# youmi-zym/GO-SLAM

Measured on NVIDIA H100. Metric: keyframe-BA-updates/s, higher is better.
Workload: dtype f16 corr (f32 accumulate) / f32 BA (f64 solve)

## Files before the change

### go-slam_b200/csrc/ba.cu

```cuda
#include "common.cuh"
#include <cstring>
#include "se3.cuh"
#include <algorithm>
#include <cstdio>
#include <mutex>
#include <cooperative_groups.h>

namespace {

constexpr int kTP = 128;
constexpr int kNRed = 27;
constexpr float kAlpha = 0.05f;

struct BaWs {
  int* slot_of_frame;
  int* kx;
  int* counts;
  int* row_ptr;
  int* edge_idx;
  int* entry_ptr;
  int* entry_code;
  int* pair_ptr;
  int* edge_j;
  float* Eij;
// ... 178 lines not shown

__device__ __forceinline__ float warp_transpose_reduce32(float (&v)[32], int lane) {
  transpose_reduce_step<16>(v, lane);
  return v[0];
}

struct BaIn {
  const float* poses; const float* disps; const float* intr; const float* disps_sens;
  const float* targets; const float* weights; const float* eta; int eta_rows;
  const int64_t* ii; const int64_t* jj;
};

__device__ __forceinline__ void linearize_tile(const BaIn& in, const BaDims& d, const BaWs& ws,
                                               int motion_only, int k, int wt) {
  const float* poses = in.poses; const float* disps = in.disps;
  const float* __restrict__ intr = in.intr; const float* __restrict__ disps_sens = in.disps_sens;
  const float* __restrict__ targets = in.targets; const float* __restrict__ weights = in.weights;
  const float* __restrict__ eta = in.eta; const int eta_rows = in.eta_rows;
  const int f = ws.kx[k];
  const int lane = threadIdx.x & 31;
  const int px = wt * 32 + lane;
  const bool act = px < d.hw;

  const float fx = intr[0], fy = intr[1], cx = intr[2], cy = intr[3];
  const float u = (float)(px % d.wd), v = (float)(px / d.wd);
  const float di = act ? disps[(size_t)f * d.hw + px] : 1.0f;
  float Xi[4] = {(u - cx) / fx, (v - cy) / fy, 1.0f, di};

  float C = 0.f, wz = 0.f;
  float Ei[6] = {0.f, 0.f, 0.f, 0.f, 0.f, 0.f};

  const int r0 = ws.row_ptr[f], r1 = ws.row_ptr[f + 1];
  float pi[7];
#pragma unroll
  for (int c = 0; c < 7; ++c) pi[c] = poses[7 * (size_t)f + c];
  int e1 = 0, j1 = f, e2 = 0, j2 = f;
  if (r0 < r1) { e1 = ws.edge_idx[r0]; j1 = ws.edge_j[e1]; }
  if (r0 + 1 < r1) { e2 = ws.edge_idx[r0 + 1]; j2 = ws.edge_j[e2]; }
  float nx[4] = {0.f, 0.f, 0.f, 0.f}, pn[7] = {0.f, 0.f, 0.f, 0.f, 0.f, 0.f, 1.f};
  if (r0 < r1) {
    if (act) {
      const size_t o = ((size_t)e1 * 2) * d.hw + px;
      nx[0] = targets[o]; nx[1] = targets[o + d.hw]; nx[2] = weights[o]; nx[3] = weights[o + d.hw];
    }
#pragma unroll
    for (int c = 0; c < 7; ++c) pn[c] = poses[7 * (size_t)j1 + c];
  }
  for (int r = r0; r < r1; ++r) {
    const int e = e1, jx = j1;
    const float tu = nx[0], tv = nx[1], qu = nx[2], qv = nx[3];
    float pj[7];
#pragma unroll
    for (int c = 0; c < 7; ++c) pj[c] = pn[c];
    e1 = e2; j1 = j2;
    if (r + 1 < r1) {
      if (act) {
        const size_t o = ((size_t)e1 * 2) * d.hw + px;
        nx[0] = targets[o]; nx[1] = targets[o + d.hw]; nx[2] = weights[o]; nx[3] = weights[o + d.hw];
      }
#pragma unroll
      for (int c = 0; c < 7; ++c) pn[c] = poses[7 * (size_t)j1 + c];
    }
    if (r + 2 < r1) { e2 = ws.edge_idx[r + 2]; j2 = ws.edge_j[e2]; }
    const bool stereo = (jx == f);
    GsSE3 G;
    if (stereo) {
      G.t[0] = -0.1f; G.t[1] = 0.f; G.t[2] = 0.f;
      G.q[0] = 0.f; G.q[1] = 0.f; G.q[2] = 0.f; G.q[3] = 1.f;
    } else {
      gs_rel(pi, pi + 3, pj, pj + 3, G);
    }

    float Xj[4];
    gs_act4(G, Xi, Xj);
    const float x = Xj[0], y = Xj[1], h = Xj[3];
    const bool behind = Xj[2] < GS_MIN_DEPTH;
    const float dd = behind ? 0.0f : __frcp_rn(Xj[2]);
    const float d2 = dd * dd;
    float wu = (behind || !act) ? 0.0f : (float)(.001 * (double)qu);
    float wv = (behind || !act) ? 0.0f : (float)(.001 * (double)qv);
    const float ru = tu - (fx * dd * x + cx);
    const float rv = tv - (fy * dd * y + cy);

    float Ju[6], Jv[6];
    Ju[0] = fx * (h * dd);       Ju[1] = fx * 0.f;
    Ju[2] = fx * (-x * h * d2);  Ju[3] = fx * (-x * y * d2);
    Ju[4] = fx * (1 + x * x * d2);  Ju[5] = fx * (-y * dd);
    Jv[0] = fy * 0.f;            Jv[1] = fy * (h * dd);
    Jv[2] = fy * (-y * h * d2);  Jv[3] = fy * (-1 - y * y * d2);
    Jv[4] = fy * (x * y * d2);   Jv[5] = fy * (x * dd);
    const float Jzu = fx * (G.t[0] * dd - G.t[2] * (x * d2));
    const float Jzv = fy * (G.t[1] * dd - G.t[2] * (y * d2));

    C += wu * Jzu * Jzu;  C += wv * Jzv * Jzv;
    wz += wu * ru * Jzu;  wz += wv * rv * Jzv;
    if (stereo) { wu = 0.f; wv = 0.f; }

    float val[32];
    {
      int l = 0;
#pragma unroll
      for (int a = 0; a < 6; ++a)
#pragma unroll
        for (int b = a; b < 6; ++b) val[l++] = wu * Ju[a] * Ju[b] + wv * Jv[a] * Jv[b];
#pragma unroll
      for (int a = 0; a < 6; ++a) val[21 + a] = wu * ru * Ju[a] + wv * rv * Jv[a];
#pragma unroll
      for (int a = kNRed; a < 32; ++a) val[a] = 0.f;
    }
    const float tot = warp_transpose_reduce32(val, lane);
    if (lane < kNRed)
      ws.part[((size_t)e * ws.ntiles * (kTP / 32) + wt) * kNRed + lane] = tot;

    if (!motion_only) {
      float Ee[6], Eii[6];
#pragma unroll
      for (int a = 0; a < 6; ++a) Ee[a] = wu * Jzu * Ju[a] + wv * Jzv * Jv[a];
      gs_adjT(G, Ee, Eii);
      if (act) {
#pragma unroll
        for (int a = 0; a < 6; ++a) {
          ws.Eij[((size_t)e * 6 + a) * d.hw + px] = Ee[a];
          Ei[a] -= Eii[a];
        }
      }
    }
  }

  if (!motion_only && act) {
    const float ds = disps_sens[(size_t)f * d.hw + px];
    const float m = (ds > 0.f) ? 1.0f : 0.0f;
    const int er = (eta_rows == 1) ? 0 : (eta_rows < 0 ? f : k);
    const float et = eta[(size_t)er * d.hw + px];
    C = C + m * kAlpha + (1.0f - m) * et;
    wz = wz - m * kAlpha * (di - ds);
    const size_t o = (size_t)k * d.hw + px;
    ws.Q[o] = 1.0f / C;
    ws.w[o] = wz;
#pragma unroll
    for (int a = 0; a < 6; ++a) ws.Ei[((size_t)k * 6 + a) * d.hw + px] = Ei[a];
  }
}

__global__ void __launch_bounds__(kTP)
ba_linearize_kernel(BaIn in, BaDims d, BaWs ws, int motion_only) {
  if ((int)blockIdx.y >= ws.counts[0] || ws.counts[4]) return;
  linearize_tile(in, d, ws, motion_only, blockIdx.y, blockIdx.x * (kTP / 32) + (threadIdx.x >> 5));
}

struct SysSmem {
  float red[8][64];
  double redd[8][32];
  double Hs[36], Ms[36], Ts[36], vs[6];
};

template <int NT>
__device__ __forceinline__ void system_items(const float* poses, const int64_t* __restrict__ ii,
                                             const int64_t* __restrict__ jj, const BaDims& d,
                                             const BaWs& ws, double* sys, int motion_only, int bid,
                                             int nb, SysSmem& sm) {
  float (*red)[64] = sm.red;
  double* Hs = sm.Hs; double* Ms = sm.Ms; double* Ts = sm.Ts; double* vs = sm.vs;
  const int tid = threadIdx.x, lane = tid & 31, warp = tid >> 5;
  const int M = ws.counts[0];
  const int npairs = motion_only ? 0 : ws.counts[2];
  constexpr int kChunk = 4 * NT;
  const int nchunk = (d.hw + kChunk - 1) / kChunk;
  double* H = sys;
  double* bvec = sys + (size_t)d.n * d.n;

  for (int e = nb - 1 - bid; e < d.N; e += nb) {
    const int ix = (int)ii[e], jx = (int)jj[e];
    const int pi = ix - d.t0, pj = jx - d.t0;
    const bool vi_ok = pi >= 0 && pi < d.P, vj_ok = pj >= 0 && pj < d.P;
    if ((!vi_ok && !vj_ok) || ix < 0 || ix >= d.num) continue;
    {
      double ps = 0.0;
      if (lane < kNRed) {
        const int nparts = ws.ntiles * (kTP / 32);
        const float* pp = ws.part + (size_t)e * nparts * kNRed + lane;
#pragma unroll 8
        for (int t = warp; t < nparts; t += NT / 32) ps += (double)pp[(size_t)t * kNRed];
      }
      sm.redd[warp][lane] = ps;
    }
    __syncthreads();
    if (tid < kNRed) {
      double s = 0.0;
#pragma unroll
      for (int wq = 0; wq < NT / 32; ++wq) s += sm.redd[wq][tid];
      if (tid < 21) {
        int a = 0, l = tid;
        while (l >= 6 - a) { l -= 6 - a; ++a; }
        const int b = a + l;
        Hs[a * 6 + b] = s; Hs[b * 6 + a] = s;
      } else {
        vs[tid - 21] = s;
      }
    }
    if (tid >= 32 && tid < 38) {
      const int c = tid - 32;
      GsSE3 G;
      gs_edge_pose(poses, ix, jx, G);
      float X[6], Y[6];
#pragma unroll
      for (int r = 0; r < 6; ++r) X[r] = (r == c) ? 1.0f : 0.0f;
      gs_adjT(G, X, Y);
#pragma unroll
      for (int r = 0; r < 6; ++r) Ms[r * 6 + c] = (double)Y[r];
    }
    __syncthreads();
    if (tid < 36) {
      const int r = tid / 6, c = tid % 6;
      double s = 0.0;
      for (int q = 0; q < 6; ++q) s += Ms[r * 6 + q] * Hs[q * 6 + c];
      Ts[tid] = s;
    }
    __syncthreads();
    if (tid < 36) {
      const int r = tid / 6, c = tid % 6;
      if (vi_ok) {
        double s = 0.0;
        for (int q = 0; q < 6; ++q) s += Ts[r * 6 + q] * Ms[c * 6 + q];
        atomicAdd(&H[(size_t)(6 * pi + r) * d.n + 6 * pi + c], s);
      }
      if (vi_ok && vj_ok) {
        atomicAdd(&H[(size_t)(6 * pi + r) * d.n + 6 * pj + c], -Ts[r * 6 + c]);
        atomicAdd(&H[(size_t)(6 * pj + r) * d.n + 6 * pi + c], -Ts[c * 6 + r]);
      }
      if (vj_ok) atomicAdd(&H[(size_t)(6 * pj + r) * d.n + 6 * pj + c], Hs[r * 6 + c]);
    } else if (tid >= 64 && tid < 70) {
      const int r = tid - 64;
      if (vj_ok) atomicAdd(&bvec[6 * pj + r], vs[r]);
      if (vi_ok) {
        double s = 0.0;
        for (int q = 0; q < 6; ++q) s += Ms[r * 6 + q] * vs[q];
        atomicAdd(&bvec[6 * pi + r], -s);
      }
    }
    __syncthreads();
  }

  const int total = npairs * nchunk;
  const int per = (total + nb - 1) / nb;
  const int u0 = bid * per;
  const int u1 = min(total, u0 + per);
  int cur = -1, pa = 0, pb = 0;
  bool diag = false;
  const float* Ea = nullptr; const float* Eb = nullptr; const float* Qk = nullptr; const float* wk = nullptr;
  float acc[64];
  auto flush = [&]() {
    float lo32[32], hi32[32];
#pragma unroll
    for (int i = 0; i < 32; ++i) { lo32[i] = acc[i]; hi32[i] = acc[32 + i]; }
    const float s0 = warp_transpose_reduce32(lo32, lane);
    const float s1 = warp_transpose_reduce32(hi32, lane);
    red[warp][lane] = s0;
    red[warp][32 + lane] = s1;
    __syncthreads();
    if (tid < 42) {
      double s = 0.0;
#pragma unroll
      for (int wq = 0; wq < NT / 32; ++wq) s += (double)red[wq][tid];
      if (tid < 36) {
        const int r = tid / 6, c = tid % 6;
        atomicAdd(&H[(size_t)(6 * pa + r) * d.n + 6 * pb + c], -s);
        if (!diag) atomicAdd(&H[(size_t)(6 * pb + c) * d.n + 6 * pa + r], -s);
      } else {
        atomicAdd(&bvec[6 * pa + (tid - 36)], -s);
      }
    }
    __syncthreads();
  };
  for (int u = u0; u < u1; ++u) {
    const int p = u / nchunk;
    const int px0 = (u - p * nchunk) * kChunk;
    const int px1 = min(d.hw, px0 + kChunk);
    if (p != cur) {
      if (cur >= 0) flush();
      cur = p;
      int k;
      if (M <= 32) {
        const int v = lane < M ? ws.pair_ptr[lane] : 0x7fffffff;
        k = __popc(__ballot_sync(0xffffffffu, v <= p)) - 1;
      } else {
        int lo = 0, hi = M;
        while (hi - lo > 1) {
          const int mid = (lo + hi) >> 1;
          if (ws.pair_ptr[mid] <= p) lo = mid; else hi = mid;
        }
        k = lo;
      }
      const int e0 = ws.entry_ptr[k];
      const int ne = ws.entry_ptr[k + 1] - e0;
      int q = p - ws.pair_ptr[k];
      int a = 0;
      while (q >= ne - a) { q -= ne - a; ++a; }
      const int b = a + q;
      const int ca = ws.entry_code[e0 + a];
      const int cb = ws.entry_code[e0 + b];
      Ea = (ca >= 0) ? ws.Eij + (size_t)ca * 6 * d.hw : ws.Ei + (size_t)k * 6 * d.hw;
      Eb = (cb >= 0) ? ws.Eij + (size_t)cb * 6 * d.hw : ws.Ei + (size_t)k * 6 * d.hw;
      pa = (ca >= 0) ? ws.edge_j[ca] - d.t0 : -ca - 1;
      pb = (cb >= 0) ? ws.edge_j[cb] - d.t0 : -cb - 1;
      Qk = ws.Q + (size_t)k * d.hw;
      wk = ws.w + (size_t)k * d.hw;
      diag = a == b;
#pragma unroll
      for (int i = 0; i < 64; ++i) acc[i] = 0.f;
    }
    float qv[kChunk / NT], wv[kChunk / NT], ea[kChunk / NT][6], eb[kChunk / NT][6];
#pragma unroll
    for (int v = 0; v < kChunk / NT; ++v) {
      const int px = px0 + tid + v * NT;
      const bool ok = px < px1;
      qv[v] = ok ? Qk[px] : 0.f;
      wv[v] = (ok && diag) ? wk[px] : 0.f;
#pragma unroll
      for (int r = 0; r < 6; ++r) {
        ea[v][r] = ok ? Ea[(size_t)r * d.hw + px] : 0.f;
        eb[v][r] = ok ? Eb[(size_t)r * d.hw + px] : 0.f;
      }
    }
#pragma unroll
    for (int v = 0; v < kChunk / NT; ++v) {
#pragma unroll
      for (int r = 0; r < 6; ++r) ea[v][r] *= qv[v];
#pragma unroll
      for (int r = 0; r < 6; ++r)
#pragma unroll
        for (int c = 0; c < 6; ++c) acc[r * 6 + c] += ea[v][r] * eb[v][c];
#pragma unroll
      for (int r = 0; r < 6; ++r) acc[36 + r] += ea[v][r] * wv[v];
    }
  }
  if (cur >= 0) flush();
}

__global__ void __launch_bounds__(256)
ba_system_kernel(const float* poses, const int64_t* __restrict__ ii,
                 const int64_t* __restrict__ jj, BaDims d, BaWs ws, int motion_only) {
  __shared__ SysSmem sm;
  if (ws.counts[4]) return;
  system_items<256>(poses, ii, jj, d, ws, ws.sys, motion_only, blockIdx.x, gridDim.x, sm);
}

constexpr int kMaxPeers = 8;
struct SysSrc {
  const double* p[kMaxPeers];
  int n;
  const unsigned* flags;
  unsigned epoch;
  int* timeout;
};
struct PeerRows {
  float* p[kMaxPeers];
  int n;
};

__device__ __forceinline__ double sys_at(const SysSrc& s, size_t i) {
  double x[kMaxPeers];
#pragma unroll
  for (int r = 0; r < kMaxPeers; ++r) x[r] = r < s.n ? __ldcg(s.p[r] + i) : 0.0;
  double v = x[0];
#pragma unroll
  for (int r = 1; r < kMaxPeers; ++r) v += x[r];
  return v;
}

__device__ __forceinline__ void peer_wait(const unsigned* flags, int n, unsigned epoch, int* timeout) {
  if (n > 1 && (int)threadIdx.x < n) {
    const long long t0 = clock64();
    unsigned v;
    do {
      asm volatile("ld.acquire.sys.global.u32 %0, [%1];" : "=r"(v) : "l"(flags + threadIdx.x) : "memory");
      if ((int)(v - epoch) >= 0) break;
      if (clock64() - t0 > (1ll << 32)) { if (timeout) *timeout = 1; break; }
    } while (true);
  }
  __syncthreads();
}

__global__ void ba_peer_wait_kernel(const unsigned* flags, int n, unsigned epoch, int* timeout) {
  peer_wait(flags, n, epoch, timeout);
}

__global__ void ba_peer_signal_kernel(PeerRows flag_rows, int slot, unsigned epoch) {
  __threadfence_system();
  if ((int)threadIdx.x < flag_rows.n) {
    unsigned* dst = reinterpret_cast<unsigned*>(flag_rows.p[threadIdx.x]) + slot;
    asm volatile("st.release.sys.global.u32 [%0], %1;" ::"l"(dst), "r"(epoch) : "memory");
  }
}

__device__ __forceinline__ void solve_finish(float* poses, const BaDims& d, const BaWs& ws,
                                             const double* x, int fail, float* dx_out,
                                             int* status_out, int tid, int nt) {
  for (int i = tid; i < d.n; i += nt) {
    const float val = fail ? 0.0f : (float)x[i];
    ws.dx[i] = val;
    if (dx_out) dx_out[i] = val;
  }
  if (tid == 0 && status_out) *status_out = fail;
}

__device__ __forceinline__ void bad_argument_step(const BaDims& d, const BaWs& ws, float* dx_out,
                                                  int* status_out, int tid, int nt) {
  for (int i = tid; i < d.n; i += nt) {
    ws.dx[i] = 0.f;
    if (dx_out) dx_out[i] = 0.f;
  }
  if (tid == 0 && status_out) *status_out = 2;
}

__device__ __forceinline__ void retract_poses(float* poses, const BaDims& d, const BaWs& ws, int tid,
                                              int nt) {
  for (int k = tid; k < d.P; k += nt) {
    float* p = poses + 7 * (size_t)(d.t0 + k);
    float t1[3], q1[4];
    gs_retr(ws.dx + 6 * k, p, p + 3, t1, q1);
    p[0] = t1[0]; p[1] = t1[1]; p[2] = t1[2];
    p[3] = q1[0]; p[4] = q1[1]; p[5] = q1[2]; p[6] = q1[3];
  }
}

struct SolveSmem {
  double Lblk[16][15];
  double xs[6];
  int failed;
};

#ifdef GOSLAM_BA_PROBE
__device__ long long g_solve_probe[8];
__device__ int g_phase_cycles[2][1024];
#define SOLVE_PROBE(slot) do { if (threadIdx.x == 0) g_solve_probe[slot] = clock64(); } while (0)
#else
#define SOLVE_PROBE(slot) do {} while (0)
#endif

__device__ __forceinline__ void solve_small(float* poses, const BaDims& d, const BaWs& ws,
                                            const SysSrc& sys_in, float lm, float ep, float* dx_out,
                                            int* status_out, double* smd, SolveSmem& ss) {
  double* xs = ss.xs;
  int& failed = ss.failed;
  const int n = d.n, P = d.P, tid = threadIdx.x, lane = tid & 31;
  double* __restrict__ A = smd;
  double* __restrict__ invd = smd + (size_t)(n + 1) * n;
  SOLVE_PROBE(0);
  float pose_old[7] = {0.f, 0.f, 0.f, 0.f, 0.f, 0.f, 1.f};
  if (tid < P) {
#pragma unroll
    for (int c = 0; c < 7; ++c) pose_old[c] = poses[7 * (size_t)(d.t0 + tid) + c];
  }
  {
    const int tot = (n + 1) * n;
    for (int base = 0; base < tot; base += 128 * 16) {
      double v[16];
#pragma unroll
      for (int u = 0; u < 16; ++u) {
        const int idx = base + tid + 128 * u;
        const int r = idx / n, c = idx - r * n;
        v[u] = (idx < tot && (c <= r || r == n)) ? sys_at(sys_in, idx) : 0.0;
      }
#pragma unroll
      for (int u = 0; u < 16; ++u) {
        const int idx = base + tid + 128 * u;
        const int r = idx / n, c = idx - r * n;
        if (idx < tot && (c <= r || r == n)) {
          double val = v[u];
          if (r == c) val += (double)ep + (double)lm * val;
          A[idx] = val;
        }
      }
    }
  }
  if (tid == 0) failed = 0;
  __syncthreads();
  SOLVE_PROBE(1);

  bool bad = false;
  for (int jb = 0; jb < P; ++jb) {
    const int j0 = 6 * jb;
    double l[6][6];
#pragma unroll
    for (int r = 0; r < 6; ++r)
#pragma unroll
      for (int c = 0; c <= r; ++c) l[r][c] = A[(j0 + r) * n + j0 + c];
#pragma unroll
    for (int k = 0; k < 6; ++k) {
      double dkk = l[k][k];
#pragma unroll
      for (int m = 0; m < k; ++m) dkk -= l[k][m] * l[k][m];
      bad = bad || !(dkk > 0.0);
      const double inv = rsqrt(dkk);
      l[k][k] = inv;
#pragma unroll
      for (int r = k + 1; r < 6; ++r) {
        double v = l[r][k];
#pragma unroll
        for (int m = 0; m < k; ++m) v -= l[r][m] * l[k][m];
        l[r][k] = v * inv;
      }
    }
    if (tid < 6) {
      invd[j0 + tid] = l[0][0] * (tid == 0) + l[1][1] * (tid == 1) + l[2][2] * (tid == 2) +
                       l[3][3] * (tid == 3) + l[4][4] * (tid == 4) + l[5][5] * (tid == 5);
    } else if (tid == 32) {
#pragma unroll
      for (int r = 1; r < 6; ++r)
#pragma unroll
        for (int c = 0; c < r; ++c) ss.Lblk[jb][r * (r - 1) / 2 + c] = l[r][c];
    }
    for (int i = j0 + 6 + tid; i <= n; i += 128) {
      double x[6];
#pragma unroll
      for (int k = 0; k < 6; ++k) x[k] = A[i * n + j0 + k];
#pragma unroll
      for (int k = 0; k < 6; ++k) {
        double v = x[k];
#pragma unroll
        for (int m = 0; m < k; ++m) v -= x[m] * l[k][m];
        x[k] = v * l[k][k];
      }
#pragma unroll
      for (int k = 0; k < 6; ++k) A[i * n + j0 + k] = x[k];
    }
    __syncthreads();
    {
      const int t4 = tid & 3;
      for (int i = j0 + 6 + (tid >> 2); i <= n; i += 32) {
        double ri[6];
#pragma unroll
        for (int k = 0; k < 6; ++k) ri[k] = A[i * n + j0 + k];
        const int cend = i < n ? i : n - 1;
        for (int c = j0 + 6 + t4; c <= cend; c += 4) {
          double acc = A[i * n + c];
#pragma unroll
          for (int k = 0; k < 6; ++k) acc -= ri[k] * A[c * n + j0 + k];
          A[i * n + c] = acc;
        }
      }
    }
    __syncthreads();
  }
  if (bad && tid == 0) failed = 1;
  __syncthreads();
  SOLVE_PROBE(2);

  double* __restrict__ y = A + (size_t)n * n;
  int fail = failed;
  if (!fail) {
    for (int jb = P - 1; jb >= 0; --jb) {
      const int j0 = 6 * jb;
      if (tid == 0) {
        double lt[6][6], x[6], iv[6];
#pragma unroll
        for (int k = 0; k < 6; ++k) { x[k] = y[j0 + k]; iv[k] = invd[j0 + k]; }
#pragma unroll
        for (int r = 1; r < 6; ++r)
#pragma unroll
          for (int c = 0; c < r; ++c) lt[r][c] = ss.Lblk[jb][r * (r - 1) / 2 + c];
#pragma unroll
        for (int k = 5; k >= 0; --k) {
          double v = x[k];
#pragma unroll
          for (int mm = k + 1; mm < 6; ++mm) v -= lt[mm][k] * x[mm];
          x[k] = v * iv[k];
        }
#pragma unroll
        for (int k = 0; k < 6; ++k) { y[j0 + k] = x[k]; xs[k] = x[k]; }
      }
      __syncthreads();
      for (int i = tid; i < j0; i += 128) {
        double v = y[i];
#pragma unroll
        for (int k = 0; k < 6; ++k) v -= A[(j0 + k) * n + i] * xs[k];
        y[i] = v;
      }
      __syncthreads();
    }
    if (tid < 32) {
      int nf = 0;
      for (int i = lane; i < n; i += 32) nf |= !isfinite(y[i]);
      if (__any_sync(0xffffffffu, nf) && lane == 0) failed = 1;
    }
    __syncthreads();
    fail = failed;
  }
  SOLVE_PROBE(3);
  solve_finish(poses, d, ws, y, fail, dx_out, status_out, tid, 128);
  if (tid < P) {
    float xi[6], t1[3], q1[4];
#pragma unroll
    for (int c = 0; c < 6; ++c) xi[c] = fail ? 0.0f : (float)y[6 * tid + c];
    gs_retr(xi, pose_old, pose_old + 3, t1, q1);
    float* p = poses + 7 * (size_t)(d.t0 + tid);
    p[0] = t1[0]; p[1] = t1[1]; p[2] = t1[2];
    p[3] = q1[0]; p[4] = q1[1]; p[5] = q1[2]; p[6] = q1[3];
  }
  SOLVE_PROBE(4);
}

__global__ void __launch_bounds__(128)
ba_solve_warp_kernel(float* poses, BaDims d, BaWs ws, const SysSrc sys_in, float lm, float ep,
                     float* dx_out, int* status_out) {
  extern __shared__ double smd[];
  __shared__ SolveSmem ss;
  if (ws.counts[4]) { bad_argument_step(d, ws, dx_out, status_out, threadIdx.x, blockDim.x); return; }
  peer_wait(sys_in.flags, sys_in.n, sys_in.epoch, sys_in.timeout);
  solve_small(poses, d, ws, sys_in, lm, ep, dx_out, status_out, smd, ss);
}

__global__ void __launch_bounds__(1024)
ba_solve_kernel(float* __restrict__ poses, BaDims d, BaWs ws, const SysSrc sys_in,
                float lm, float ep, int use_smem, float* __restrict__ dx_out,
                int* __restrict__ status_out) {
  extern __shared__ double smd[];
  __shared__ int fail;
  const int n = d.n, tid = threadIdx.x, nt = blockDim.x;
  if (ws.counts[4]) { bad_argument_step(d, ws, dx_out, status_out, tid, nt); return; }
  peer_wait(sys_in.flags, sys_in.n, sys_in.epoch, sys_in.timeout);
  double* A = use_smem ? smd : ws.chol;
  double* b = use_smem ? smd + (size_t)n * n : ws.rhs;
  if (tid == 0) fail = 0;
  for (size_t idx = tid; idx < (size_t)n * n; idx += nt) {
    const int r = (int)(idx / n), c = (int)(idx % n);
    double val = sys_at(sys_in, idx);
    if (r == c) val += (double)ep + (double)lm * val;
    A[idx] = val;
  }
  for (int i = tid; i < n; i += nt) b[i] = sys_at(sys_in, (size_t)n * n + i);
  __syncthreads();

  for (int j = 0; j < n; ++j) {
    const double ajj = A[(size_t)j * n + j];
    if (!(ajj > 0.0)) { if (tid == 0) fail = 1; }
    __syncthreads();
    if (fail) break;
    const double inv = rsqrt(ajj);
    for (int i = j + 1 + tid; i < n; i += nt) A[(size_t)i * n + j] *= inv;
    if (tid == 0) A[(size_t)j * n + j] = inv;
    __syncthreads();
    const int m = n - j - 1;
    const int tot = m * m;
    for (int idx = tid; idx < tot; idx += nt) {
      const int q = idx / m;
      const int i = j + 1 + q, c = j + 1 + (idx - q * m);
      if (c <= i) A[(size_t)i * n + c] -= A[(size_t)i * n + j] * A[(size_t)c * n + j];
    }
    __syncthreads();
  }

  if (!fail) {
    for (int j = 0; j < n; ++j) {
      const double zj = b[j] * A[(size_t)j * n + j];
      __syncthreads();
      if (tid == 0) b[j] = zj;
      for (int i = j + 1 + tid; i < n; i += nt) b[i] -= A[(size_t)i * n + j] * zj;
      __syncthreads();
    }
    for (int j = n - 1; j >= 0; --j) {
      const double xj = b[j] * A[(size_t)j * n + j];
      __syncthreads();
      if (tid == 0) b[j] = xj;
      for (int i = tid; i < j; i += nt) b[i] -= A[(size_t)j * n + i] * xj;
      __syncthreads();
    }
    int bad = 0;
    for (int i = tid; i < n; i += nt) bad |= !isfinite(b[i]);
    if (bad) fail = 1;
    __syncthreads();
  }
  solve_finish(poses, d, ws, b, fail, dx_out, status_out, tid, nt);
  __syncthreads();
  retract_poses(poses, d, ws, tid, nt);
}

constexpr int kCl = 8;
constexpr int kClT = 512;

__host__ __device__ inline int cl_row_off(int q, int l) {
  return 36 * (l * (q + 1) + kCl * (l * (l - 1) / 2));
}
inline size_t cl_rows_doubles(int P) {
  size_t mx = 0;
  for (int q = 0; q < kCl; ++q) {
    const int nl = (P - q + kCl - 1) / kCl;
    if (nl > 0) mx = std::max(mx, (size_t)cl_row_off(q, nl));
  }
  return mx;
}
inline size_t cl_smem_bytes(int P) {
// ... 274 lines not shown
    __shared__ int any_fail;
    if (tid == 0) {
      int f = 0;
      for (int oq = 0; oq < kCl; ++oq) f |= *cluster.map_shared_rank(&failed, oq);
      any_fail = f;
    }
    __syncthreads();
    const int fail = any_fail;
    for (int i = tid; i < n; i += kClT) {
      const float val = fail ? 0.0f : ws.dx[i];
      ws.dx[i] = val;
      if (dx_out) dx_out[i] = val;
    }
    if (tid == 0 && status_out) *status_out = fail;
    __syncthreads();
    retract_poses(poses, d, ws, tid, kClT);
  }
  cluster.sync();
}

__device__ __forceinline__ void backsub_tile(float* disps, const BaDims& d, const BaWs& ws,
                                             int owner_lo, int owner_hi, float* dz_out, int k,
                                             int wt, const PeerRows* peers = nullptr) {
  const int f = ws.kx[k];
  if (f < owner_lo || f >= owner_hi) return;
  const int px = wt * 32 + (threadIdx.x & 31);
  if (px >= d.hw) return;
  float acc = 0.f;
  {
    const int ix = f - d.t0;
    if (ix > 0 && ix < d.P) {
      float dw = 0.f;
#pragma unroll
      for (int a = 0; a < 6; ++a) dw += ws.Ei[((size_t)k * 6 + a) * d.hw + px] * ws.dx[6 * ix + a];
      acc += dw;
    }
  }
  for (int r = ws.row_ptr[f]; r < ws.row_ptr[f + 1]; ++r) {
    const int e = ws.edge_idx[r];
    const int ix = ws.edge_j[e] - d.t0;
    if (ix <= 0 || ix >= d.P) continue;
    float dw = 0.f;
#pragma unroll
    for (int a = 0; a < 6; ++a) dw += ws.Eij[((size_t)e * 6 + a) * d.hw + px] * ws.dx[6 * ix + a];
    acc += dw;
  }
  const size_t o = (size_t)k * d.hw + px;
  const float dz = ws.Q[o] * (ws.w[o] - acc);
  const float nv = disps[(size_t)f * d.hw + px] + dz;
  disps[(size_t)f * d.hw + px] = nv;
  if (peers)
    for (int r = 0; r < peers->n; ++r)
      if (peers->p[r] != disps) peers->p[r][(size_t)f * d.hw + px] = nv;
  if (dz_out) dz_out[(size_t)f * d.hw + px] = dz;
}

__global__ void __launch_bounds__(kTP)
ba_backsub_kernel(float* disps, BaDims d, BaWs ws, int owner_lo, int owner_hi, float* dz_out, const PeerRows peers) {
  if ((int)blockIdx.y >= ws.counts[0] || ws.counts[4]) return;
  backsub_tile(disps, d, ws, owner_lo, owner_hi, dz_out, blockIdx.y, blockIdx.x * (kTP / 32) + (threadIdx.x >> 5),
               peers.n > 1 ? &peers : nullptr);
}

#ifdef GOSLAM_BA_PROBE
#define BA_PROBE(slot) do { if (threadIdx.x == 0 && blockIdx.x == 0) probe[slot] = clock64(); } while (0)
#else
#define BA_PROBE(slot) do {} while (0)
#endif

__device__ __forceinline__ void block_arrive(unsigned* counter) {
  __syncthreads();
  if (threadIdx.x == 0) {
    __threadfence();
    atomicAdd(counter, 1u);
  }
}

__device__ __forceinline__ void block_wait_at_least(const unsigned* word, unsigned target) {
  if (threadIdx.x == 0) {
    unsigned v;
    do {
      asm volatile("ld.acquire.gpu.global.u32 %0, [%1];" : "=r"(v) : "l"(word) : "memory");
    } while (v < target);
    __threadfence();
  }
  __syncthreads();
}

__device__ __forceinline__ void block_publish(unsigned* word, unsigned value) {
  __syncthreads();
  if (threadIdx.x == 0) {
    __threadfence();
    asm volatile("st.release.gpu.global.u32 [%0], %1;" ::"l"(word), "r"(value) : "memory");
  }
}

__device__ __forceinline__ void grid_barrier(unsigned* counter, unsigned& epoch) {
  block_arrive(counter);
  ++epoch;
  block_wait_at_least(counter, epoch * gridDim.x);
}

__global__ void __launch_bounds__(kTP)
ba_persistent_kernel(float* poses, float* disps, BaIn in, BaDims d, BaWs ws, int iterations, float lm,
                     float ep, int motion_only, float* dx_out, float* dz_out, int* status_out,
                     unsigned* barrier, unsigned* arrived, unsigned* solved) {
  extern __shared__ double smd[];
  __shared__ SysSmem sys_sm;
  __shared__ SolveSmem solve_sm;
  unsigned epoch = 0;
#ifdef GOSLAM_BA_PROBE
  __shared__ long long probe[8];
#endif
  const int M = ws.counts[0];
  const int nwt = ws.ntiles * (kTP / 32);
  const int units = M * nwt;
  const int ufirst = (threadIdx.x >> 5) * gridDim.x + blockIdx.x, ustep = (kTP / 32) * gridDim.x;
  const size_t nsys = (size_t)d.n * d.n + d.n;
  if (dz_out) {
    const size_t ndz = (size_t)d.num * d.hw;
    for (size_t i = (size_t)blockIdx.x * kTP + threadIdx.x; i < ndz; i += (size_t)gridDim.x * kTP) dz_out[i] = 0.f;
  }
  if (ws.counts[4]) {
    if (blockIdx.x == 0) {
      bad_argument_step(d, ws, dx_out, nullptr, threadIdx.x, kTP);
      if (status_out) for (int it = threadIdx.x; it < iterations; it += kTP) status_out[it] = 2;
    }
    return;
  }
  for (int it = 0; it < iterations; ++it) {
    BA_PROBE(0);
#ifdef GOSLAM_BA_PROBE
    const long long tl0 = clock64();
#endif
    double* const sys = (it & 1) ? ws.sys_alt : ws.sys;
    for (int u = ufirst; u < units; u += ustep) {
      const int k = u / nwt, wt = u - k * nwt;
      if (it > 0 && !motion_only) backsub_tile(disps, d, ws, 0, d.num, dz_out, k, wt);
      linearize_tile(in, d, ws, motion_only, k, wt);
    }
    if (it + 1 < iterations) {
      double* const next = (it & 1) ? ws.sys : ws.sys_alt;
      for (size_t i = (size_t)blockIdx.x * kTP + threadIdx.x; i < nsys; i += (size_t)gridDim.x * kTP) next[i] = 0.0;
    }
#ifdef GOSLAM_BA_PROBE
    if (threadIdx.x == 0 && blockIdx.x < 1024) g_phase_cycles[0][blockIdx.x] = (int)(clock64() - tl0);
#endif
    BA_PROBE(1);
    grid_barrier(barrier, epoch);
    BA_PROBE(2);
#ifdef GOSLAM_BA_PROBE
    const long long ts0 = clock64();
#endif
    system_items<kTP>(poses, in.ii, in.jj, d, ws, sys, motion_only, blockIdx.x, gridDim.x, sys_sm);
#ifdef GOSLAM_BA_PROBE
    if (threadIdx.x == 0 && blockIdx.x < 1024) g_phase_cycles[1][blockIdx.x] = (int)(clock64() - ts0);
#endif
    BA_PROBE(3);
    block_arrive(arrived);
    if (blockIdx.x == 0) {
      block_wait_at_least(arrived, (unsigned)(it + 1) * gridDim.x);
      BA_PROBE(4);
      SysSrc local{};
      local.p[0] = sys; local.n = 1;
      solve_small(poses, d, ws, local, lm, ep, dx_out, status_out ? status_out + it : nullptr, smd,
                  solve_sm);
      BA_PROBE(5);
      block_publish(solved, it + 1);
    } else {
      block_wait_at_least(solved, it + 1);
    }
    BA_PROBE(6);
#ifdef GOSLAM_BA_PROBE
    if (threadIdx.x == 0 && blockIdx.x == 0 && it == iterations - 1) {
      for (int ph = 0; ph < 2; ++ph) {
        int mx = 0, arg = 0;
        for (int b = 0; b < (int)gridDim.x && b < 1024; ++b)
          if (g_phase_cycles[ph][b] > mx) { mx = g_phase_cycles[ph][b]; arg = b; }
        printf("[phase %d] slowest block %d: %d cycles; blocks 0/100/200/244/250/270/290/295: %d %d %d %d %d %d %d %d\n", ph, arg,
               mx, g_phase_cycles[ph][0], g_phase_cycles[ph][100], g_phase_cycles[ph][200], g_phase_cycles[ph][244],
               g_phase_cycles[ph][250], g_phase_cycles[ph][270], g_phase_cycles[ph][290], g_phase_cycles[ph][295]);
      }
    }
    if (threadIdx.x == 0 && blockIdx.x == 0)
      printf("[solve probe it=%d] load %lld | factor %lld | backward %lld | finish+retract %lld\n", it,
             g_solve_probe[1] - g_solve_probe[0], g_solve_probe[2] - g_solve_probe[1],
             g_solve_probe[3] - g_solve_probe[2], g_solve_probe[4] - g_solve_probe[3]);
    if (threadIdx.x == 0 && blockIdx.x == 0)
      printf("[ba probe it=%d] linearize %lld | barrier %lld | system %lld | wait for arrivals %lld | solve %lld | publish %lld (cycles)\n",
             it, probe[1] - probe[0], probe[2] - probe[1], probe[3] - probe[2], probe[4] - probe[3],
             probe[5] - probe[4], probe[6] - probe[5]);
#endif
  }
  if (!motion_only)
    for (int u = ufirst; u < units; u += ustep) {
      const int k = u / nwt, wt = u - k * nwt;
      backsub_tile(disps, d, ws, 0, d.num, dz_out, k, wt);
    }
}

bool make_dims(int N, int num, int ht, int wd, int t0, int t1, BaDims* d) {
  if (N < 0 || num <= 0 || num > 4096 || ht <= 0 || wd <= 0) return false;
  d->N = N; d->num = num; d->ht = ht; d->wd = wd; d->hw = ht * wd;
  d->t0 = t0; d->t1 = t1; d->P = t1 - t0 > 0 ? t1 - t0 : 0; d->n = 6 * d->P;
  if (t0 < 0 || t1 > num) return false;
  return true;
}

constexpr int kSmemSolveMaxN = 160;
constexpr int kWarpSolveMaxN = 96;
constexpr int kMaxDevices = 64;
constexpr size_t kClusterSmemMax = 226 * 1024;

struct BaDevice {
  bool ready = false;
  int sms = 0;
  int blocks_per_sm = 0;
};

void ba_persistent_kernel_attrs(BaDevice* dv, int dev) {
  int occ = 0, coop = 0;
  const size_t smem_max = ((size_t)kWarpSolveMaxN * kWarpSolveMaxN + 2 * kWarpSolveMaxN) * sizeof(double);
  cudaDeviceGetAttribute(&dv->sms, cudaDevAttrMultiProcessorCount, dev);
  cudaDeviceGetAttribute(&coop, cudaDevAttrCooperativeLaunch, dev);
  cudaFuncSetAttribute(ba_persistent_kernel, cudaFuncAttributeMaxDynamicSharedMemorySize, (int)smem_max);
  cudaOccupancyMaxActiveBlocksPerMultiprocessor(&occ, ba_persistent_kernel, kTP, smem_max);
#ifndef GOSLAM_BA_BLOCKS_PER_SM
#define GOSLAM_BA_BLOCKS_PER_SM 2
#endif
  constexpr int kWant = GOSLAM_BA_BLOCKS_PER_SM;
  dv->blocks_per_sm = (!coop || occ < 1) ? 0 : (occ > kWant ? kWant : occ);
}

inline size_t prep_smem_bytes(int num) { return ((size_t)3 * num + 1 + 33) * sizeof(int); }

const BaDevice& ba_device() {
  static BaDevice table[kMaxDevices];
  static std::mutex mu;
  int dev = 0;
  cudaGetDevice(&dev);
  if (dev < 0 || dev >= kMaxDevices) dev = 0;
  std::lock_guard<std::mutex> lock(mu);
  BaDevice& dv = table[dev];
  if (!dv.ready) {
    cudaFuncSetAttribute(ba_prep_kernel, cudaFuncAttributeMaxDynamicSharedMemorySize, (int)prep_smem_bytes(kPrepMaxFrames));
    cudaFuncSetAttribute(ba_solve_kernel, cudaFuncAttributeMaxDynamicSharedMemorySize,
                         (int)(((size_t)kSmemSolveMaxN * kSmemSolveMaxN + kSmemSolveMaxN) * 8));
    cudaFuncSetAttribute(ba_solve_warp_kernel, cudaFuncAttributeMaxDynamicSharedMemorySize,
                         (int)(((size_t)kWarpSolveMaxN * kWarpSolveMaxN + 2 * kWarpSolveMaxN) * 8));
    cudaFuncSetAttribute(ba_solve_cluster_kernel, cudaFuncAttributeMaxDynamicSharedMemorySize,
                         (int)kClusterSmemMax);
    ba_persistent_kernel_attrs(&dv, dev);
    dv.ready = true;
  }
  return dv;
}


int launch_phase1(const float* poses, const float* disps, const float* intr,
                  const float* disps_sens, const float* targets, const float* weights,
                  const float* eta, int eta_rows, const int64_t* ii, const int64_t* jj,
                  const BaDims& d, const BaWs& ws, int motion_only, bool prep, cudaStream_t st) {
  const BaIn in{poses, disps, intr, disps_sens, targets, weights, eta, eta_rows, ii, jj};
  if (prep) {
    ba_prep_kernel<<<1, kPrepThreads, prep_smem_bytes(d.num), st>>>(ii, jj, d, ws, 0, motion_only ? 0 : eta_rows);
    GS_CHECK_LAUNCH();
  }
  cudaMemsetAsync(ws.sys, 0, ((size_t)d.n * d.n + d.n) * sizeof(double), st);
  if (d.N > 0) {
    dim3 grid(ws.ntiles, d.num);
    ba_linearize_kernel<<<grid, kTP, 0, st>>>(in, d, ws, motion_only);
    GS_CHECK_LAUNCH();
  } else if (!motion_only) {
    dim3 grid(ws.ntiles, d.num);
    ba_linearize_kernel<<<grid, kTP, 0, st>>>(in, d, ws, motion_only);
    GS_CHECK_LAUNCH();
  }
  ba_system_kernel<<<kNumSms * 4, 256, 0, st>>>(poses, ii, jj, d, ws, motion_only);
  GS_CHECK_LAUNCH();
  return GOSLAM_OK;
}

int launch_phase2(float* poses, float* disps, const SysSrc& sys_in,
                  const BaDims& d, const BaWs& ws, float lm, float ep, int motion_only,
                  int owner_lo, int owner_hi, float* dx_out, float* dz_out, int* status_out,
                  cudaStream_t st, const PeerRows& peer_rows = PeerRows{}) {
  const BaDevice& dv = ba_device();
  (void)dv;
  if (d.n <= kWarpSolveMaxN) {
    const size_t smem = ((size_t)d.n * d.n + 2 * d.n) * sizeof(double);
    ba_solve_warp_kernel<<<1, 128, smem, st>>>(poses, d, ws, sys_in, lm, ep, dx_out, status_out);
  } else if (cl_smem_bytes(d.P) <= kClusterSmemMax) {
    cudaLaunchConfig_t cfg = {};
    cfg.gridDim = dim3(kCl);
    cfg.blockDim = dim3(kClT);
    cfg.dynamicSmemBytes = cl_smem_bytes(d.P);
    cfg.stream = st;
    cudaLaunchAttribute attr[1];
    attr[0].id = cudaLaunchAttributeClusterDimension;
    attr[0].val.clusterDim.x = kCl; attr[0].val.clusterDim.y = 1; attr[0].val.clusterDim.z = 1;
    cfg.attrs = attr;
    cfg.numAttrs = 1;
    const int rows_doubles = (int)cl_rows_doubles(d.P);
    const cudaError_t le = cudaLaunchKernelEx(&cfg, ba_solve_cluster_kernel, poses, d, ws, sys_in, lm, ep,
                                              rows_doubles, dx_out, status_out);
    if (le != cudaSuccess) { gs_note_cuda_error(le); return GOSLAM_ELAUNCH; }
  } else {
// ... 238 lines not shown
```

Baseline: 1767.

## Pipeline next diagonal Cholesky factor with trailing update and cache pair decode

In the blocked Cholesky, warp 0 now updates the next diagonal 6x6 block and factors it while the other warps do the rest of the trailing update. This takes the serial diagonal factorisation off the critical path between iterations, and the trailing update is register-blocked across three columns. Separately, the pair-index decode in system_items is cached in shared memory on the first BA iteration and reused on later ones, which avoids the search and global lookups. The reuse depends on every block seeing the same pair schedule each iteration, and the factor state is now shared through smem, which brings extra syncs and more complex index logic.

Result: no change. 1757, median of 6 (-0.6%).

```diff
diff --git a/go-slam_b200/csrc/ba.cu b/go-slam_b200/csrc/ba.cu
--- a/go-slam_b200/csrc/ba.cu
+++ b/go-slam_b200/csrc/ba.cu
@@ -354,13 +354,15 @@
   float red[8][64];
   double redd[8][32];
   double Hs[36], Ms[36], Ts[36], vs[6];
+  int pairs[4][7];
 };
+constexpr int kPairCache = 4;
 
 template <int NT>
 __device__ __forceinline__ void system_items(const float* poses, const int64_t* __restrict__ ii,
                                              const int64_t* __restrict__ jj, const BaDims& d,
                                              const BaWs& ws, double* sys, int motion_only, int bid,
-                                             int nb, SysSmem& sm) {
+                                             int nb, SysSmem& sm, int pair_cache = 0) {
   float (*red)[64] = sm.red;
   double* Hs = sm.Hs; double* Ms = sm.Ms; double* Ts = sm.Ts; double* vs = sm.vs;
   const int tid = threadIdx.x, lane = tid & 31, warp = tid >> 5;
@@ -447,7 +449,7 @@
   const int per = (total + nb - 1) / nb;
   const int u0 = bid * per;
   const int u1 = min(total, u0 + per);
-  int cur = -1, pa = 0, pb = 0;
+  int cur = -1, pa = 0, pb = 0, npair = 0;
   bool diag = false;
   const float* Ea = nullptr; const float* Eb = nullptr; const float* Qk = nullptr; const float* wk = nullptr;
   float acc[64];
@@ -481,33 +483,43 @@
     if (p != cur) {
       if (cur >= 0) flush();
       cur = p;
-      int k;
-      if (M <= 32) {
-        const int v = lane < M ? ws.pair_ptr[lane] : 0x7fffffff;
-        k = __popc(__ballot_sync(0xffffffffu, v <= p)) - 1;
+      const int slot = npair++;
+      int k, ca, cb;
+      if (pair_cache == 2 && slot < kPairCache && sm.pairs[slot][0] == p) {
+        k = sm.pairs[slot][1]; ca = sm.pairs[slot][2]; cb = sm.pairs[slot][3];
+        pa = sm.pairs[slot][4]; pb = sm.pairs[slot][5]; diag = sm.pairs[slot][6];
       } else {
-        int lo = 0, hi = M;
-        while (hi - lo > 1) {
-          const int mid = (lo + hi) >> 1;
-          if (ws.pair_ptr[mid] <= p) lo = mid; else hi = mid;
+        if (M <= 32) {
+          const int v = lane < M ? ws.pair_ptr[lane] : 0x7fffffff;
+          k = __popc(__ballot_sync(0xffffffffu, v <= p)) - 1;
+        } else {
+          int lo = 0, hi = M;
+          while (hi - lo > 1) {
+            const int mid = (lo + hi) >> 1;
+            if (ws.pair_ptr[mid] <= p) lo = mid; else hi = mid;
+          }
+          k = lo;
         }
-        k = lo;
-      }
-      const int e0 = ws.entry_ptr[k];
-      const int ne = ws.entry_ptr[k + 1] - e0;
-      int q = p - ws.pair_ptr[k];
-      int a = 0;
-      while (q >= ne - a) { q -= ne - a; ++a; }
-      const int b = a + q;
-      const int ca = ws.entry_code[e0 + a];
-      const int cb = ws.entry_code[e0 + b];
+        const int e0 = ws.entry_ptr[k];
+        const int ne = ws.entry_ptr[k + 1] - e0;
+        int q = p - ws.pair_ptr[k];
+        int a = 0;
+        while (q >= ne - a) { q -= ne - a; ++a; }
+        const int b = a + q;
+        ca = ws.entry_code[e0 + a];
+        cb = ws.entry_code[e0 + b];
+        pa = (ca >= 0) ? ws.edge_j[ca] - d.t0 : -ca - 1;
+        pb = (cb >= 0) ? ws.edge_j[cb] - d.t0 : -cb - 1;
+        diag = a == b;
+        if (pair_cache == 1 && slot < kPairCache && tid == 0) {
+          sm.pairs[slot][0] = p; sm.pairs[slot][1] = k; sm.pairs[slot][2] = ca; sm.pairs[slot][3] = cb;
+          sm.pairs[slot][4] = pa; sm.pairs[slot][5] = pb; sm.pairs[slot][6] = diag;
+        }
+      }
       Ea = (ca >= 0) ? ws.Eij + (size_t)ca * 6 * d.hw : ws.Ei + (size_t)k * 6 * d.hw;
       Eb = (cb >= 0) ? ws.Eij + (size_t)cb * 6 * d.hw : ws.Ei + (size_t)k * 6 * d.hw;
-      pa = (ca >= 0) ? ws.edge_j[ca] - d.t0 : -ca - 1;
-      pb = (cb >= 0) ? ws.edge_j[cb] - d.t0 : -cb - 1;
       Qk = ws.Q + (size_t)k * d.hw;
       wk = ws.w + (size_t)k * d.hw;
-      diag = a == b;
 #pragma unroll
       for (int i = 0; i < 64; ++i) acc[i] = 0.f;
     }
@@ -640,6 +652,40 @@
 #define SOLVE_PROBE(slot) do {} while (0)
 #endif
 
+__device__ __forceinline__ bool solve_small_factor_diag(const double* A, int n, int jb, double* invd,
+                                                        SolveSmem& ss) {
+  const int j0 = 6 * jb;
+  double l[6][6];
+  bool bad = false;
+#pragma unroll
+  for (int r = 0; r < 6; ++r)
+#pragma unroll
+    for (int c = 0; c <= r; ++c) l[r][c] = A[(j0 + r) * n + j0 + c];
+#pragma unroll
+  for (int k = 0; k < 6; ++k) {
+    double dkk = l[k][k];
+#pragma unroll
+    for (int m = 0; m < k; ++m) dkk -= l[k][m] * l[k][m];
+    bad = bad || !(dkk > 0.0);
+    const double inv = rsqrt(dkk);
+    l[k][k] = inv;
+#pragma unroll
+    for (int r = k + 1; r < 6; ++r) {
+      double v = l[r][k];
+#pragma unroll
+      for (int m = 0; m < k; ++m) v -= l[r][m] * l[k][m];
+      l[r][k] = v * inv;
+    }
+  }
+#pragma unroll
+  for (int k = 0; k < 6; ++k) invd[j0 + k] = l[k][k];
+#pragma unroll
+  for (int r = 1; r < 6; ++r)
+#pragma unroll
+    for (int c = 0; c < r; ++c) ss.Lblk[jb][r * (r - 1) / 2 + c] = l[r][c];
+  return !bad;
+}
+
 __device__ __forceinline__ void solve_small(float* poses, const BaDims& d, const BaWs& ws,
                                             const SysSrc& sys_in, float lm, float ep, float* dx_out,
                                             int* status_out, double* smd, SolveSmem& ss) {
@@ -681,39 +727,18 @@
   SOLVE_PROBE(1);
 
   bool bad = false;
+  if (tid == 0) bad = !solve_small_factor_diag(A, n, 0, invd, ss);
+  __syncthreads();
   for (int jb = 0; jb < P; ++jb) {
     const int j0 = 6 * jb;
-    double l[6][6];
-#pragma unroll
-    for (int r = 0; r < 6; ++r)
-#pragma unroll
-      for (int c = 0; c <= r; ++c) l[r][c] = A[(j0 + r) * n + j0 + c];
-#pragma unroll
-    for (int k = 0; k < 6; ++k) {
-      double dkk = l[k][k];
-#pragma unroll
-      for (int m = 0; m < k; ++m) dkk -= l[k][m] * l[k][m];
-      bad = bad || !(dkk > 0.0);
-      const double inv = rsqrt(dkk);
-      l[k][k] = inv;
-#pragma unroll
-      for (int r = k + 1; r < 6; ++r) {
-        double v = l[r][k];
-#pragma unroll
-        for (int m = 0; m < k; ++m) v -= l[r][m] * l[k][m];
-        l[r][k] = v * inv;
-      }
-    }
-    if (tid < 6) {
-      invd[j0 + tid] = l[0][0] * (tid == 0) + l[1][1] * (tid == 1) + l[2][2] * (tid == 2) +
-                       l[3][3] * (tid == 3) + l[4][4] * (tid == 4) + l[5][5] * (tid == 5);
-    } else if (tid == 32) {
-#pragma unroll
-      for (int r = 1; r < 6; ++r)
-#pragma unroll
-        for (int c = 0; c < r; ++c) ss.Lblk[jb][r * (r - 1) / 2 + c] = l[r][c];
-    }
     for (int i = j0 + 6 + tid; i <= n; i += 128) {
+      double l[6][6];
+#pragma unroll
+      for (int k = 0; k < 6; ++k) {
+        l[k][k] = invd[j0 + k];
+#pragma unroll
+        for (int m = 0; m < k; ++m) l[k][m] = ss.Lblk[jb][k * (k - 1) / 2 + m];
+      }
       double x[6];
 #pragma unroll
       for (int k = 0; k < 6; ++k) x[k] = A[i * n + j0 + k];
@@ -728,18 +753,43 @@
       for (int k = 0; k < 6; ++k) A[i * n + j0 + k] = x[k];
     }
     __syncthreads();
-    {
+    if (jb + 1 == P) break;
+    if (tid < 32) {
+      if (lane < 21) {
+        int r = 0, c = lane;
+        while (c > r) { c -= r + 1; ++r; }
+        const int i = j0 + 6 + r, cc = j0 + 6 + c;
+        double acc = A[i * n + cc];
+#pragma unroll
+        for (int k = 0; k < 6; ++k) acc -= A[i * n + j0 + k] * A[cc * n + j0 + k];
+        A[i * n + cc] = acc;
+      }
+      __syncwarp();
+      if (lane == 0) bad = !solve_small_factor_diag(A, n, jb + 1, invd, ss) || bad;
+    } else {
+      constexpr int kB = 3;
       const int t4 = tid & 3;
-      for (int i = j0 + 6 + (tid >> 2); i <= n; i += 32) {
+      for (int i = j0 + 12 + ((tid - 32) >> 2); i <= n; i += 24) {
         double ri[6];
 #pragma unroll
         for (int k = 0; k < 6; ++k) ri[k] = A[i * n + j0 + k];
         const int cend = i < n ? i : n - 1;
-        for (int c = j0 + 6 + t4; c <= cend; c += 4) {
-          double acc = A[i * n + c];
-#pragma unroll
-          for (int k = 0; k < 6; ++k) acc -= ri[k] * A[c * n + j0 + k];
-          A[i * n + c] = acc;
+        for (int c = j0 + 6 + t4; c <= cend; c += 4 * kB) {
+          double acc[kB], lc[kB][6];
+#pragma unroll
+          for (int q = 0; q < kB; ++q) {
+            const int cq = c + 4 * q <= cend ? c + 4 * q : c;
+            acc[q] = A[i * n + cq];
+#pragma unroll
+            for (int k = 0; k < 6; ++k) lc[q][k] = A[cq * n + j0 + k];
+          }
+#pragma unroll
+          for (int q = 0; q < kB; ++q)
+#pragma unroll
+            for (int k = 0; k < 6; ++k) acc[q] -= ri[k] * lc[q][k];
+#pragma unroll
+          for (int q = 0; q < kB; ++q)
+            if (c + 4 * q <= cend) A[i * n + c + 4 * q] = acc[q];
         }
       }
     }
@@ -1320,7 +1370,7 @@
 #ifdef GOSLAM_BA_PROBE
     const long long ts0 = clock64();
 #endif
-    system_items<kTP>(poses, in.ii, in.jj, d, ws, sys, motion_only, blockIdx.x, gridDim.x, sys_sm);
+    system_items<kTP>(poses, in.ii, in.jj, d, ws, sys, motion_only, blockIdx.x, gridDim.x, sys_sm, it == 0 ? 1 : 2);
 #ifdef GOSLAM_BA_PROBE
     if (threadIdx.x == 0 && blockIdx.x < 1024) g_phase_cycles[1][blockIdx.x] = (int)(clock64() - ts0);
 #endif
```
